# kevlar-dev/kevlar

Measured on AMD Instinct MI355X. Metric: reads/sec through count+novel (3 samples, k=31), higher is better.
Workload: dtype u64 hash / u8 counters

## Files before the change

### kevlar_amd/csrc/kv_skm.hip

```cpp
#include <algorithm>
#include <cmath>

#include "kv_binned.h"
#include "kv_novel_device.h"
#include "kv_skm_device.h"

struct SkmGeom {
    int k, m, w, wpow;
    int kw, nbw, recw, ncap;
    uint32_t C1, F2, fbits;
    uint32_t nwg1, nwg2, quota1;
    uint32_t cap1, cap2;
    uint32_t np_max;
    uint64_t stride;
    uint64_t *seg1; uint32_t *cnt1;
    uint64_t *seg2; uint32_t *cnt2;
    uint64_t *loose; uint64_t loose_cap;
    unsigned long long *ctr;
    uint32_t n_buckets, quota3;
    uint32_t sbw;
    uint64_t bucket_kmers;
    uint32_t force_loose;
    uint64_t *abl_keys; uint8_t *abl_cnts; uint32_t *abl_bstart, *abl_bcount; uint32_t abl_cap_wg;
    uint64_t *dl_keys, *dl_hash; uint32_t *dl_bstart, *dl_bcount; uint32_t dl_cap_wg;
// ... 636 lines not shown
        auto append = [&](unsigned long long bal, uint32_t v, uint32_t lane_start, uint32_t end) -> bool {
            const uint32_t slot = __builtin_amdgcn_mbcnt_hi((uint32_t)(bal >> 32), __builtin_amdgcn_mbcnt_lo((uint32_t)bal, n_ent));
            if (slot >= SKM_LANE_CAP) return false;
            ent[slot] = (unsigned long long)v | ((unsigned long long)(lane_start | (end << 18)) << 32);
            return true;
        };
        auto flush = [&]() {
            if (!pf_waited) {
#pragma unroll
                for (int i = 0; i < NW; ++i) asm volatile("" : "+v"(pf[i]));
                pf_waited = true;
            }
            __builtin_amdgcn_fence(__ATOMIC_ACQ_REL, "wavefront");
            __builtin_amdgcn_wave_barrier();
            const uint32_t n = min(n_ent, SKM_LANE_CAP);
            for (uint32_t e = lane; e < n; e += 64u) {
                const unsigned long long en = ent[e];
                const uint32_t hi = (uint32_t)(en >> 32), first = (hi >> 6) & 4095u;
                emit_run((uint32_t)en, hi & 63u, first, (hi >> 18) - first);
            }
            __builtin_amdgcn_fence(__ATOMIC_ACQ_REL, "wavefront");
            __builtin_amdgcn_wave_barrier();
            n_ent = 0;
        };
        uint32_t Sa[B], Sb[B];
#pragma unroll
        for (int j = 0; j < B; ++j) { Sa[j] = 0xffffffffu; Sb[j] = 0xffffffffu; }
        uint32_t prev_v = 0, start_prev = 0;
        const uint32_t rbase = lane * wpr;
        uint32_t since = 0;
        for (uint32_t b = 0; b < nblocks; b += (C == 2 ? 2u : 1u)) {
            skm_lane_block<C>(wl, rbase, lane, b, npos, nk, Sa, Sb, prev_v, start_prev, n_ent, append);
            if (C == 2 && b + 1u < nblocks) skm_lane_block<C>(wl, rbase, lane, b + 1u, npos, nk, Sb, Sa, prev_v, start_prev, n_ent, append);
            since += (C == 2 ? 2u : 1u);
            if ((since >= flush_blocks || n_ent + 192u > SKM_LANE_CAP) && n_ent && b + (C == 2 ? 2u : 1u) < nblocks) { flush(); since = 0; }
        }
        if (n_ent + 64u > SKM_LANE_CAP) flush();
        {
            const unsigned long long bal = __ballot(active);
            if (active) (void)append(bal, prev_v, start_prev, nk);
            n_ent += (uint32_t)__popcll(bal);
        }
        flush();
    }
    __syncthreads();
    for (uint32_t c = threadIdx.x; c < sg.C1; c += SKM_LANE_THREADS) sg.cnt1[skm_seg1_slot(sg, c, blockIdx.x)] = min(cur[c], sg.cap1);
    n_rec = wave_sum_u64(n_rec);
    if ((threadIdx.x & 63u) == 0 && n_rec) atomicAdd(&sg.ctr[SKM_CTR_RECORDS], (unsigned long long)n_rec);
}

#define SKM_THREADS2 512
#define SKM_MAX_F2 4096u
template <bool COMPACT>
__global__ __launch_bounds__(SKM_THREADS2) void k_skm_split(SkmGeom sg)
{
    __shared__ uint32_t cur[SKM_MAX_F2];
    __shared__ uint32_t spre[769];
    const uint32_t c = blockIdx.y;
    for (uint32_t f = threadIdx.x; f < sg.F2; f += SKM_THREADS2) cur[f] = 0;
    const uint32_t nmine = (skm_seg1_count(sg) - blockIdx.x + sg.nwg2 - 1) / sg.nwg2;
    for (uint32_t i = threadIdx.x; i < nmine; i += SKM_THREADS2) spre[i + 1] = sg.cnt1[skm_seg1_slot(sg, c, blockIdx.x + i * sg.nwg2)];
    __syncthreads();
    if (threadIdx.x == 0) {
        uint32_t acc = 0;
        for (uint32_t i = 0; i < nmine; ++i) { const uint32_t n = spre[i + 1]; spre[i] = acc; acc += n; }
        spre[nmine] = acc;
    }
    __syncthreads();
    const uint32_t total = spre[nmine];
    const int recw = COMPACT ? 2 : sg.recw;
    for (uint32_t i = threadIdx.x; i < total; i += SKM_THREADS2) {
        const uint32_t si = skm_search(spre, nmine, i);
        const uint32_t seg = blockIdx.x + si * sg.nwg2;
        const uint64_t *rec = sg.seg1 + (skm_seg1_first(sg, skm_seg1_slot(sg, c, seg)) + (i - spre[si])) * (uint64_t)recw;
        if (COMPACT) {
            typedef uint64_t u64x2a __attribute__((ext_vector_type(2), aligned(16)));
            const u64x2a both = *(const u64x2a *)rec;
            const uint32_t fine = skm_c_fine(both.y);
            const uint32_t p = atomicAdd(&cur[fine], 1u);
            if (p < sg.cap2) {
                *(u64x2a *)(sg.seg2 + ((((uint64_t)c * sg.F2 + fine) * sg.nwg2 + blockIdx.x) * sg.cap2 + p) * 2ull) = both;
            } else {
                uint64_t lw[3] = {both.x, skm_c_b1(both.y), 0ull};
                skm_loose_push(sg, skm_header(0ull, skm_c_n(both.y), fine, skm_c_rev(both.y)), lw);
            }
            continue;
        }
        const uint64_t hdr = rec[0];
        uint64_t bw[3];
#pragma unroll
        for (int t = 0; t < 3; ++t) bw[t] = t < sg.nbw ? rec[1 + t] : 0ull;
        const uint32_t fine = skm_hdr_fine(hdr);
        const uint32_t p = atomicAdd(&cur[fine], 1u);
        if (p < sg.cap2)
            skm_store_record(sg.seg2 + ((((uint64_t)c * sg.F2 + fine) * sg.nwg2 + blockIdx.x) * sg.cap2 + p) * (uint64_t)recw, hdr, bw, sg.nbw);
        else skm_loose_push(sg, hdr, bw);
    }
    __syncthreads();
    for (uint32_t f = threadIdx.x; f < sg.F2; f += SKM_THREADS2)
        sg.cnt2[((uint64_t)c * sg.F2 + f) * sg.nwg2 + blockIdx.x] = min(cur[f], sg.cap2);
}

#define SKM_S2_CHUNK 2048u
#define SKM_S2_MAXF 1024u
template <int RECW>
__global__ __launch_bounds__(SKM_THREADS2) void k_skm_split_sorted(SkmGeom sg)
{
    __shared__ uint32_t cur[SKM_S2_MAXF];
    __shared__ uint32_t hist[SKM_S2_MAXF];
    __shared__ uint32_t off[SKM_S2_MAXF];
    __shared__ uint32_t spre[769];
    __shared__ uint32_t wsum[SKM_THREADS2 / 64];
    extern __shared__ __attribute__((aligned(16))) uint64_t img[];
    const uint32_t c = blockIdx.y, F2 = sg.F2;
    const uint32_t lane = threadIdx.x & 63u, wave = threadIdx.x >> 6;
    for (uint32_t f = threadIdx.x; f < F2; f += SKM_THREADS2) { cur[f] = 0; hist[f] = 0; }
    const uint32_t nmine = (skm_seg1_count(sg) - blockIdx.x + sg.nwg2 - 1) / sg.nwg2;
    for (uint32_t i = threadIdx.x; i < nmine; i += SKM_THREADS2) spre[i + 1] = sg.cnt1[skm_seg1_slot(sg, c, blockIdx.x + i * sg.nwg2)];
    __syncthreads();
    if (threadIdx.x == 0) {
        uint32_t acc = 0;
        for (uint32_t i = 0; i < nmine; ++i) { const uint32_t n = spre[i + 1]; spre[i] = acc; acc += n; }
        spre[nmine] = acc;
    }
    __syncthreads();
    const uint32_t total = spre[nmine];
    constexpr uint32_t PER = SKM_S2_CHUNK / SKM_THREADS2;
    const uint32_t fper = (F2 + SKM_THREADS2 - 1) / SKM_THREADS2;
    uint64_t *const out = sg.seg2 + ((uint64_t)c * F2 * sg.nwg2 + blockIdx.x) * sg.cap2 * RECW;
    const uint64_t fstride = (uint64_t)sg.nwg2 * sg.cap2 * RECW;
    uint64_t nh[PER], n0[PER], n1[PER], n2[PER];
    auto request = [&](uint32_t c0) {
        const uint32_t n = c0 < total ? min(SKM_S2_CHUNK, total - c0) : 0u;
#pragma unroll
        for (uint32_t r = 0; r < PER; ++r) {
            const uint32_t i = r * SKM_THREADS2 + threadIdx.x;
            nh[r] = 0; n0[r] = 0; n1[r] = 0; n2[r] = 0;
            if (i < n) {
                const uint32_t gi = c0 + i, si = skm_search(spre, nmine, gi);
                const uint32_t seg = blockIdx.x + si * sg.nwg2;
                const uint64_t *rec = sg.seg1 + (skm_seg1_first(sg, skm_seg1_slot(sg, c, seg)) + (gi - spre[si])) * (uint64_t)RECW;
                if (RECW == 2) {
                    typedef uint64_t u64x2a __attribute__((ext_vector_type(2), aligned(16)));
                    const u64x2a both = *(const u64x2a *)rec;
                    n0[r] = both.x; nh[r] = both.y;
                } else {
                    nh[r] = rec[0]; n0[r] = rec[1]; n1[r] = rec[2];
                    if (RECW == 4) n2[r] = rec[3];
                }
            }
        }
    };
    request(0);
    for (uint32_t c0 = 0; c0 < total; c0 += SKM_S2_CHUNK) {
        const uint32_t n = min(SKM_S2_CHUNK, total - c0);
        uint64_t hdr[PER], w0[PER], w1[PER], w2[PER];
        uint32_t rank[PER];
#pragma unroll
        for (uint32_t r = 0; r < PER; ++r) { hdr[r] = nh[r]; w0[r] = n0[r]; w1[r] = n1[r]; w2[r] = n2[r]; rank[r] = 0; }
        request(c0 + SKM_S2_CHUNK);
#pragma unroll
        for (uint32_t r = 0; r < PER; ++r)
            if (r * SKM_THREADS2 + threadIdx.x < n) rank[r] = atomicAdd(&hist[RECW == 2 ? skm_c_fine(hdr[r]) : skm_hdr_fine(hdr[r])], 1u);
        __syncthreads();
        {
            uint32_t h[2] = {0, 0}, sum = 0;
            for (uint32_t j = 0; j < fper; ++j) {
                const uint32_t f = threadIdx.x * fper + j;
                h[j] = f < F2 ? hist[f] : 0u;
                sum += h[j];
            }
            uint32_t incl = sum;
#pragma unroll
            for (int d = 1; d < 64; d <<= 1) {
                const uint32_t up = __shfl_up(incl, d);
                if (lane >= (uint32_t)d) incl += up;
            }
            if (lane == 63) wsum[wave] = incl;
            __syncthreads();
            uint32_t before = incl - sum;
            for (uint32_t wv = 0; wv < wave; ++wv) before += wsum[wv];
            for (uint32_t j = 0; j < fper; ++j) {
                const uint32_t f = threadIdx.x * fper + j;
                if (f < F2) {
                    off[f] = before;
                    const uint32_t at = cur[f];
                    cur[f] = at + h[j];
                    hist[f] = at - before;
                    before += h[j];
                }
            }
        }
        __syncthreads();
#pragma unroll
        for (uint32_t r = 0; r < PER; ++r) {
            if (r * SKM_THREADS2 + threadIdx.x < n) {
                uint64_t *dst = img + (uint64_t)(off[RECW == 2 ? skm_c_fine(hdr[r]) : skm_hdr_fine(hdr[r])] + rank[r]) * RECW;
                if (RECW == 2) { dst[0] = w0[r]; dst[1] = hdr[r]; }
                else { dst[0] = hdr[r]; dst[1] = w0[r]; dst[2] = w1[r]; }
                if (RECW == 4) dst[3] = w2[r];
            }
        }
        __syncthreads();
        for (uint32_t wd = threadIdx.x; wd < n * RECW; wd += SKM_THREADS2) {
            const uint32_t q = wd / RECW, part = wd - q * RECW;
            const uint64_t h0 = img[(uint64_t)q * RECW + (RECW == 2 ? 1 : 0)];
            const uint32_t f = RECW == 2 ? skm_c_fine(h0) : skm_hdr_fine(h0);
            const uint32_t slot = q + hist[f];
            if (slot < sg.cap2) out[(uint64_t)f * fstride + (uint64_t)slot * RECW + part] = img[wd];
            else if (part == 0) {
                if (RECW == 2) {
                    uint64_t bw[3] = {img[(uint64_t)q * RECW], skm_c_b1(h0), 0ull};
                    skm_loose_push(sg, skm_header(0ull, skm_c_n(h0), f, skm_c_rev(h0)), bw);
                } else {
                    uint64_t bw[3] = {img[(uint64_t)q * RECW + 1], img[(uint64_t)q * RECW + 2], RECW == 4 ? img[(uint64_t)q * RECW + 3] : 0ull};
                    skm_loose_push(sg, h0, bw);
                }
            }
        }
        __syncthreads();
        for (uint32_t f = threadIdx.x; f < F2; f += SKM_THREADS2) hist[f] = 0;
        __syncthreads();
    }
    for (uint32_t f = threadIdx.x; f < F2; f += SKM_THREADS2)
        sg.cnt2[((uint64_t)c * F2 + f) * sg.nwg2 + blockIdx.x] = min(cur[f], sg.cap2);
}

#define SKM_STEP_MASK 62u
#define SKM_PROBE_STEP(h) ((((h) >> 20) & SKM_STEP_MASK) | 1u)
template <int TS>
__device__ __forceinline__ uint32_t skm_slot0(uint32_t sh) { return (TS & (TS - 1)) == 0 ? sh & (uint32_t)(TS - 1) : __umulhi(sh, (uint32_t)TS); }
template <int TS>
__device__ __forceinline__ uint32_t skm_step_of(uint32_t sh) { return (TS & (TS - 1)) == 0 ? SKM_PROBE_STEP(sh) : (((sh >> 2) & 62u) | 1u); }
template <int TS>
__device__ __forceinline__ uint32_t skm_slot_next(uint32_t slot, uint32_t step)
{
    if ((TS & (TS - 1)) == 0) return (slot + step) & (uint32_t)(TS - 1);
    slot += step;
    return slot >= (uint32_t)TS ? slot - (uint32_t)TS : slot;
}
template <int KW, int TS>
struct SkmTable {
    unsigned long long key[KW][TS];
};

template <int KW, int TS>
__device__ __forceinline__ void skm_table_clear(SkmTable<KW, TS> &tb)
{
    for (uint32_t i = threadIdx.x; i < TS; i += blockDim.x) {
        tb.key[0][i] = SKM_EMPTY;
        if (KW == 2) tb.key[KW - 1][i] = SKM_EMPTY;
    }
}

template <int KW, int TS>
__device__ __forceinline__ int skm_table_insert(SkmTable<KW, TS> &tb, const SkmKey<KW> &c)
{
    const uint32_t sh = skm_slot_hash<KW>(c);
    uint32_t slot = skm_slot0<TS>(sh);
    const uint32_t step = skm_step_of<TS>(sh);
    for (int probe = 0; probe < SKM_MAXPROBE; ++probe) {
        const unsigned long long old0 = atomicCAS(&tb.key[0][slot], SKM_EMPTY, (unsigned long long)c.w[0]);
        if (old0 == SKM_EMPTY || old0 == c.w[0]) {
            if (KW == 1) return (int)slot;
            const unsigned long long old1 = atomicCAS(&tb.key[KW - 1][slot], SKM_EMPTY, (unsigned long long)c.w[KW - 1]);
            if (old1 == SKM_EMPTY || old1 == c.w[KW - 1]) return (int)slot;
        }
        slot = skm_slot_next<TS>(slot, step);
    }
    return -1;
}

template <int KW, int TS>
__device__ __forceinline__ int skm_table_find(const SkmTable<KW, TS> &tb, const SkmKey<KW> &c)
{
    const uint32_t sh = skm_slot_hash<KW>(c);
    uint32_t slot = skm_slot0<TS>(sh);
    const uint32_t step = skm_step_of<TS>(sh);
    for (int probe = 0; probe < SKM_MAXPROBE; ++probe) {
        const unsigned long long k0 = tb.key[0][slot];
        if (k0 == SKM_EMPTY) return -1;
        if (k0 == c.w[0] && (KW == 1 || tb.key[KW - 1][slot] == c.w[KW - 1])) return (int)slot;
        slot = skm_slot_next<TS>(slot, step);
    }
    return -1;
}

template <typename Emit>
__device__ __forceinline__ uint32_t skm_count_kmer(uint64_t h, uint32_t count, const SketchDev *__restrict__ sk,
                                                   const SketchDev *__restrict__ mask, const ConsumeFilter &f, int T, Emit emit)
{
    if (!consume_filter_pass(f, mask, h)) return 0;
    uint32_t left = min(count, 255u);
    while (left) {
        const uint32_t wgt = min(left, BIN_W_MAX);
#pragma unroll
        for (int t = 0; t < BIN_MAX_T; ++t)
            if (t < T) emit(t, fastmod(h, sk->size[t], sk->magic[t]), wgt);
        left -= wgt;
    }
    return count;
}

template <int TS, typename Body>
__device__ __forceinline__ void skm_for_occupied(const unsigned long long *key0, uint16_t *queue_all, uint32_t queue_stride, Body body, const uint32_t *skip = nullptr)
{
    const uint32_t wave = threadIdx.x >> 6, lane = threadIdx.x & 63, nwaves = blockDim.x >> 6;
    uint16_t *queue = queue_all + wave * queue_stride;
    const uint32_t per_wave = TS / nwaves;
    const uint32_t s_end = (wave + 1) * per_wave;
    uint32_t qn = 0;
    for (uint32_t s0 = wave * per_wave;; s0 += 64) {
        const bool last = s0 >= s_end;
        if (!last) {
            const uint32_t slot = s0 + lane;
            const bool occ = key0[slot] != SKM_EMPTY && !(skip && ((skip[slot >> 5] >> (slot & 31u)) & 1u));
            const unsigned long long ballot = __ballot(occ);
            if (occ) __hip_atomic_store(&queue[qn + (uint32_t)__popcll(ballot & ((1ull << lane) - 1ull))], (uint16_t)slot, __ATOMIC_RELAXED, __HIP_MEMORY_SCOPE_WAVEFRONT);
            qn += (uint32_t)__popcll(ballot);
            __builtin_amdgcn_fence(__ATOMIC_ACQ_REL, "wavefront");
            __builtin_amdgcn_wave_barrier();
        }
        if (qn >= 64 || (last && qn > 0)) {
            const uint32_t take = min(qn, 64u);
            qn -= take;
            if (lane < take) body((uint32_t)__hip_atomic_load(&queue[qn + lane], __ATOMIC_RELAXED, __HIP_MEMORY_SCOPE_WAVEFRONT));
            __builtin_amdgcn_fence(__ATOMIC_ACQ_REL, "wavefront");
            __builtin_amdgcn_wave_barrier();
        }
        if (last) break;
    }
}

#define SKM_UNIT 4

__device__ __forceinline__ uint64_t skm_shfl64(uint64_t v, uint32_t src)
{
    const uint32_t lo = (uint32_t)__shfl((int)(uint32_t)v, (int)src), hi = (uint32_t)__shfl((int)(uint32_t)(v >> 32), (int)src);
    return (uint64_t)lo | ((uint64_t)hi << 32);
}

template <int KW>
__device__ __forceinline__ SkmKey<KW> skm_kmer_at(uint64_t b0, uint64_t b1, uint64_t b2, uint32_t j, int k)
{
    return skm_kmer_of<KW>(b0, b1, b2, j, k);
}

template <int KW, bool WANT_POS>
__device__ __forceinline__ void skm_walk_loose(const SkmGeom &sg, bool alone, const SkmKey<KW> &kmer, uint64_t hdr, uint32_t owner,
                                               uint64_t pos0, uint32_t j0, uint32_t u, uint32_t lane, int recw)
{
    const unsigned long long need = __ballot(alone);
    if (!need) return;
    const uint64_t posu = WANT_POS ? pos0 : skm_hdr_pos_of(skm_shfl64(hdr, owner), j0 + u);
    unsigned long long first = 0;
    if (lane == 0) first = atomicAdd(&sg.ctr[SKM_CTR_LOOSE], (unsigned long long)__popcll(need));
    first = skm_shfl64(first, 0);
    if (alone) {
        const unsigned long long idx = first + (unsigned long long)__popcll(need & ((1ull << lane) - 1ull));
        uint64_t one[3] = {kmer.w[0], KW == 2 ? kmer.w[KW - 1] : 0ull, 0ull};
        if (idx < sg.loose_cap) skm_store_record(sg.loose + idx * (uint64_t)recw, skm_header(posu, 1u, 0u), one, sg.nbw);
        else sg.ctr[SKM_CTR_FAIL] = 1;
    }
}

template <int KW, bool WANT_POS, int FK = 0, bool COMPACT = false, typename Body>
__device__ __forceinline__ void skm_walk_bucket(const SkmGeom &sg, uint32_t b, uint32_t *sbits_all, Body body)
{
    static_assert(!COMPACT || (KW == 1 && !WANT_POS), "compact records: one-word keys, no positions");
    constexpr uint32_t G = SKM_UNIT;
    const uint32_t lane = threadIdx.x & 63, wave = threadIdx.x >> 6, nwaves = blockDim.x >> 6;
    uint32_t *sbits = sbits_all + wave * sg.sbw;
    const int k = FK ? FK : sg.k, recw = COMPACT ? 2 : (FK ? 1 + KW + 1 : sg.recw);
    auto load = [&](const uint64_t *rec, uint64_t &hdr, uint64_t &b0, uint64_t &b1, uint64_t &b2) {
        if (COMPACT) {
            typedef uint64_t u64x2a __attribute__((ext_vector_type(2), aligned(16)));
            const u64x2a both = *(const u64x2a *)rec;
            b0 = both.x; b1 = skm_c_b1(both.y); hdr = skm_header(0ull, skm_c_n(both.y), 0u, skm_c_rev(both.y));
        } else {
            hdr = rec[0]; b0 = rec[1]; b1 = rec[2];
            if (KW == 2) b2 = rec[3];
        }
    };
    const uint32_t *cnt2 = sg.cnt2 + (uint64_t)b * sg.nwg2;
    uint32_t p = wave;
    uint32_t g = p / sg.nwg2, sgm = p - g * sg.nwg2;
    uint64_t hdr = 0, b0 = 0, b1 = 0, b2 = 0;
    {
        const uint32_t at = min(g * 64u + lane, sg.cap2 - 1u);
        const uint64_t *rec = sg.seg2 + (((uint64_t)b * sg.nwg2 + sgm) * sg.cap2 + at) * (uint64_t)recw;
        load(rec, hdr, b0, b1, b2);
    }
    uint32_t maxc = 0;
    for (uint32_t s2 = 0; s2 < sg.nwg2; ++s2) maxc = max(maxc, cnt2[s2]);
    for (;;) {
        if (g * 64u >= maxc) break;
        const uint32_t NR = cnt2[sgm], i = g * 64u + lane;
        const uint32_t nk = i < NR ? skm_hdr_n(hdr) : 0u;
        const uint32_t nu = (nk + G - 1u) / G;
        uint32_t incl = nu;
#pragma unroll
        for (int d = 1; d < 64; d <<= 1) {
            const uint32_t up = __shfl_up(incl, d);
            if (lane >= d) incl += up;
        }
        const uint32_t total = __shfl(incl, 63), excl = incl - nu;
        const uint32_t exnk = excl | (nk << 16);
        const uint32_t nwords = (total >> 5) + 2u;
        for (uint32_t wd = lane; wd < nwords; wd += 64) sbits[wd] = 0;
        __builtin_amdgcn_fence(__ATOMIC_RELEASE, "wavefront");
        __builtin_amdgcn_wave_barrier();
        if (nu) atomicOr(&sbits[excl >> 5], 1u << (excl & 31));
        __builtin_amdgcn_fence(__ATOMIC_ACQ_REL, "wavefront");
        __builtin_amdgcn_wave_barrier();
        uint32_t before = 0;
        for (uint32_t t0 = 0; t0 < total; t0 += 64) {
            const uint64_t starts = (uint64_t)__hip_atomic_load(&sbits[t0 >> 5], __ATOMIC_RELAXED, __HIP_MEMORY_SCOPE_WAVEFRONT) |
                                    ((uint64_t)__hip_atomic_load(&sbits[(t0 >> 5) + 1], __ATOMIC_RELAXED, __HIP_MEMORY_SCOPE_WAVEFRONT) << 32);
            const uint32_t t = t0 + lane;
            const uint32_t owner = (before + (uint32_t)__popcll(starts & ((2ull << lane) - 1ull)) - 1u) & 63u;
            before += (uint32_t)__popcll(starts);
            const uint32_t oe = (uint32_t)__shfl((int)exnk, (int)owner);
            const uint64_t o0 = skm_shfl64(b0, owner), o1 = skm_shfl64(b1, owner);
            const uint64_t o2 = KW == 2 ? skm_shfl64(b2, owner) : 0ull;
            const uint64_t oh = WANT_POS ? skm_shfl64(hdr, owner) : 0ull;
            const uint32_t j0 = t < total ? (t - (oe & 0xffffu)) * G : 0u;
            const uint32_t cnt = t < total ? min(G, (oe >> 16) - j0) : 0u;
            SkmKey<KW> fw = skm_kmer_of<KW>(o0, o1, o2, j0, k);
            const uint32_t tail = (uint32_t)skm_window64(o0, o1, o2, j0 + (uint32_t)k);
            uint64_t pos0 = 0;
            int step = 1;
            if (WANT_POS) {
                const bool rv = skm_hdr_rev(oh) != 0u;
                pos0 = skm_hdr_pos(oh) + (rv ? skm_hdr_n(oh) - 1u - j0 : j0);
                step = rv ? -1 : 1;
            }
#pragma unroll
            for (uint32_t u = 0; u < G; ++u) {
                if (u) { SkmKey<KW> other = fw; skm_roll<KW>(fw, other, (tail >> (2u * (u - 1u))) & 3u, k); }
                const uint64_t posu = pos0 + (uint64_t)(int64_t)(step * (int)u);
                bool alone = false;
                if (u < cnt) alone = body(fw, posu);
                skm_walk_loose<KW, WANT_POS>(sg, alone, fw, hdr, owner, posu, j0, u, lane, sg.lrecw);
            }
        }
        __builtin_amdgcn_wave_barrier();
        p += nwaves;
        g = p / sg.nwg2; sgm = p - g * sg.nwg2;
        if (g * 64u >= maxc) break;
        if (g * 64u + lane < cnt2[sgm]) {
            const uint64_t *rec = sg.seg2 + (((uint64_t)b * sg.nwg2 + sgm) * sg.cap2 + g * 64u + lane) * (uint64_t)recw;
            load(rec, hdr, b0, b1, b2);
        }
    }
}

__host__ __device__ inline uint32_t skm_wave_scratch_words(uint32_t sbw) { return sbw > 64u ? sbw : 64u; }

#define SKM_K2_WAVES 6
#define SKM_TS51 2560
#define SKM_TS31 4096
#define SKM_LIST_MAX 4096u
template <int KW, int TS, bool FORCE_LOOSE, int FK, bool COMPACT = false>
__global__ __launch_bounds__(SKM_THREADS3, KW == 2 ? SKM_K2_WAVES : 6) void k_skm_count(SkmGeom sg, const SketchDev *__restrict__ sk,
                                                           const SketchDev *__restrict__ mask, ConsumeFilter f, BinGeom g)
{
    static_assert((uint32_t)TS <= SKM_LIST_MAX, "a bucket's distinct list (one entry per occupied slot) must fit what k_skm_novel_list takes");
    constexpr bool PL = FK != 0;
    __shared__ SkmTable<KW, TS> tb;
    __shared__ uint32_t cnt[PL ? TS / 2 : TS];
    __shared__ uint32_t next_bucket;
    __shared__ uint32_t abl_cur, abl_b0, abl_prev;
    __shared__ uint32_t dl_cur, dl_b0;
    extern __shared__ __attribute__((aligned(16))) uint32_t dyn[];
    const uint32_t ns = (uint32_t)(g.T * g.C);
    uint32_t *lut = dyn, *cur = dyn + (PL ? 1024 : 256), *scratch = cur + ((ns + 3u) & ~3u);
    uint64_t *P1 = (uint64_t *)dyn, *P2 = P1 + 256;
    for (uint32_t s = threadIdx.x; s < ns; s += SKM_THREADS3) cur[s] = 0;
    if (threadIdx.x < 256) {
        if (PL) { P1[threadIdx.x] = skm_ascii4_times(threadIdx.x, MM_C1); P2[threadIdx.x] = skm_ascii4_times(threadIdx.x, MM_C2); }
        else lut[threadIdx.x] = skm_ascii4(threadIdx.x);
    }
    const HashParams hp = FK ? make_hash_params(FK, f.hp.hashfam) : f.hp;
    uint64_t n_added = 0, n_distinct = 0;
    const uint32_t cap1 = (uint32_t)g.cap1;
    uint32_t *my_seg = g.gbuf1 + (uint64_t)blockIdx.x * g.cap1;
    const uint64_t seg_stride = (uint64_t)g.nwgA * g.cap1;
    auto emit = [&](int t, uint64_t bin, uint32_t wgt) {
        const uint32_t slice = (uint32_t)(bin >> g.sbits);
        const uint32_t c = g.F == 1 ? slice : __umulhi(slice, g.recipF);
        const uint32_t sidx = (uint32_t)t * (uint32_t)g.C + c;
        const uint32_t item = ((slice - c * (uint32_t)g.F) << g.sbits) | ((uint32_t)bin & ((1u << g.sbits) - 1u)) | ((wgt - 1u) << BIN_W_SHIFT);
        const uint32_t pos = atomicAdd(&cur[sidx], 1u);
        if (pos < cap1) my_seg[sidx * seg_stride + pos] = item;
        else spill_item(g, t, bin, wgt);
    };
    skm_table_clear(tb);
    for (uint32_t i = threadIdx.x; i < (PL ? TS / 2 : TS); i += SKM_THREADS3) cnt[i] = 0;
    if (threadIdx.x == 0) { next_bucket = (uint32_t)atomicAdd(&sg.ctr[SKM_CTR_TICKET_COUNT], 1ull) * sg.bpt; abl_cur = 0; abl_b0 = 0; abl_prev = 0xffffffffu; dl_cur = 0; dl_b0 = 0; }
    auto abl_close = [&]() {
        if (sg.abl_keys && abl_prev != 0xffffffffu) {
            const bool fits = abl_cur <= sg.abl_cap_wg;
            sg.abl_bstart[abl_prev] = blockIdx.x * sg.abl_cap_wg + abl_b0;
            sg.abl_bcount[abl_prev] = fits ? abl_cur - abl_b0 : 0u;
        }
        if (sg.dl_keys && abl_prev != 0xffffffffu) {
            sg.dl_bstart[abl_prev] = blockIdx.x * sg.dl_cap_wg + dl_b0;
            sg.dl_bcount[abl_prev] = dl_cur - dl_b0;
        }
    };
    for (uint32_t taken = 0; taken < sg.quota3; ++taken) {
        __syncthreads();
        const uint32_t b = next_bucket;
        if (b >= sg.n_buckets) break;
        __syncthreads();
        if (threadIdx.x == 0) {
            abl_close();
            abl_prev = b; abl_b0 = abl_cur; dl_b0 = dl_cur;
            if ((b + 1u) & (sg.bpt - 1u)) next_bucket = b + 1u;
            else if (taken + 1 >= sg.quota3 || __hip_atomic_load(&sg.ctr[SKM_CTR_FAIL], __ATOMIC_RELAXED, __HIP_MEMORY_SCOPE_AGENT) != 0) next_bucket = 0xffffffffu;
            else {
                const unsigned long long ticket = atomicAdd(&sg.ctr[SKM_CTR_TICKET_COUNT], 1ull);
                next_bucket = (uint32_t)ticket * sg.bpt;
                const unsigned long long done = ticket * sg.bpt;
                if (done * 50ull >= sg.n_buckets) {
                    const unsigned long long now = __hip_atomic_load(&sg.ctr[SKM_CTR_LOOSE], __ATOMIC_RELAXED, __HIP_MEMORY_SCOPE_AGENT), start = sg.ctr[SKM_CTR_LOOSE_S12];
                    if (now > start && (now - start) * 25ull > done * sg.bucket_kmers) sg.ctr[SKM_CTR_FAIL] = 1;
                }
            }
        }
        skm_walk_bucket<KW, false, FK, COMPACT>(sg, b, scratch, [&](const SkmKey<KW> &c, uint64_t) {
            const bool forced = FORCE_LOOSE && sg.force_loose && ((c.w[0] * 0x9e3779b97f4a7c15ull) >> 58) == 0;
            const int slot = skm_cacheable<KW>(c) && !forced ? skm_table_insert(tb, c) : -1;
            if (slot >= 0) {
                if (PL) atomicAdd(&cnt[(uint32_t)slot >> 1], 1u << (((uint32_t)slot & 1u) * 16u));
                else atomicAdd(&cnt[slot], 1u);
            }
            return slot < 0;
        });
        __syncthreads();
        skm_for_occupied<TS>(tb.key[0], (uint16_t *)scratch, skm_wave_scratch_words(sg.sbw) * 2u, [&](uint32_t slot) {
            SkmKey<KW> c;
            c.w[0] = tb.key[0][slot];
            tb.key[0][slot] = SKM_EMPTY;
            if (KW == 2) { c.w[KW - 1] = tb.key[KW - 1][slot]; tb.key[KW - 1][slot] = SKM_EMPTY; }
            uint32_t seen;
            if (PL) {
                const uint32_t sh = (slot & 1u) * 16u;
                seen = (cnt[slot >> 1] >> sh) & 0xffffu;
                atomicSub(&cnt[slot >> 1], seen << sh);
            } else {
                seen = cnt[slot];
                cnt[slot] = 0;
            }
            n_distinct += 1;
            uint64_t h;
            if constexpr (PL) h = skm_key_hash_pl<KW, FK>(c, P1, P2);
            else h = skm_key_hash<KW>(c, lut, hp);
            if (sg.dl_keys) {
                const unsigned long long here = __ballot(true);
                const uint32_t lane = threadIdx.x & 63u, leader = (uint32_t)__ffsll((long long)here) - 1u;
                uint32_t base = 0;
                if (lane == leader) base = atomicAdd(&dl_cur, (uint32_t)__popcll(here));
                base = (uint32_t)__shfl((int)base, (int)leader);
                const uint32_t at = base + (uint32_t)__popcll(here & ((1ull << lane) - 1ull));
                if (at < sg.dl_cap_wg) {
                    const uint64_t e = (uint64_t)blockIdx.x * sg.dl_cap_wg + at;
                    sg.dl_keys[e * KW] = c.w[0];
                    if (KW == 2) sg.dl_keys[e * KW + (KW - 1)] = c.w[KW - 1];
                    sg.dl_hash[e] = h;
                }
            }
            uint32_t added;
            if (g.fast4 && !f.use_mask) {
                const bool pass = !f.use_band || (h >= f.band_lo && h < f.band_hi);
                added = pass ? seen : 0u;
                if (pass) {
                    const double hd = kv_fastmod_hd(h);
                    uint32_t bin[4];
#pragma unroll
                    for (int t = 0; t < 4; ++t) bin[t] = kv_fastmod32(h, hd, (uint32_t)g.tsize[t], g.tmagic[t]);
                    uint32_t left = min(seen, 255u);
                    const uint32_t omask = (1u << g.sbits) - 1u, stride32 = (uint32_t)seg_stride;
                    while (left) {
                        const uint32_t wgt = min(left, BIN_W_MAX), wbits = (wgt - 1u) << BIN_W_SHIFT;
#pragma unroll
                        for (int t = 0; t < 4; ++t) {
                            const uint32_t slice = bin[t] >> g.sbits;
                            const uint32_t c = g.F == 1 ? slice : __umulhi(slice, g.recipF);
                            const uint32_t sidx = (uint32_t)t * (uint32_t)g.C + c;
                            const uint32_t item = ((slice - c * (uint32_t)g.F) << g.sbits) | (bin[t] & omask) | wbits;
                            const uint32_t pos = atomicAdd(&cur[sidx], 1u);
                            if (pos < cap1) my_seg[sidx * stride32 + pos] = item;
                            else spill_item(g, t, (uint64_t)bin[t], wgt);
                        }
                        left -= wgt;
                    }
                }
            } else {
                added = skm_count_kmer(h, seen, sk, mask, f, g.T, emit);
            }
            n_added += added;
            if (sg.abl_keys) {
                const bool want = added >= 2u;
                const unsigned long long here = __ballot(true), vote = __ballot(want);
                if (vote) {
                    const uint32_t lane = threadIdx.x & 63u, leader = (uint32_t)__ffsll((long long)here) - 1u;
                    uint32_t base = 0;
                    if (lane == leader) base = atomicAdd(&abl_cur, (uint32_t)__popcll(vote));
                    base = (uint32_t)__shfl((int)base, (int)leader);
                    const uint32_t at = base + (uint32_t)__popcll(vote & ((1ull << lane) - 1ull));
                    if (want && at < sg.abl_cap_wg) {
                        const uint64_t e = (uint64_t)blockIdx.x * sg.abl_cap_wg + at;
                        sg.abl_keys[e * KW] = c.w[0];
                        if (KW == 2) sg.abl_keys[e * KW + (KW - 1)] = c.w[KW - 1];
                        sg.abl_cnts[e] = (uint8_t)min(added, 255u);
                    }
                }
            }
        });
    }
    __syncthreads();
    if (threadIdx.x == 0) {
        abl_close();
        if (sg.dl_keys && dl_cur > sg.dl_cap_wg) atomicAdd(&sg.ctr[SKM_CTR_DL_RAN_OUT], 1ull);
    }
    for (uint32_t s = threadIdx.x; s < ns; s += SKM_THREADS3)
        g.gcnt1[(uint64_t)s * g.nwgA + blockIdx.x] = (uint32_t)min((uint64_t)cur[s], g.cap1);
    n_added = wave_sum_u64(n_added);
    n_distinct = wave_sum_u64(n_distinct);
    if ((threadIdx.x & 63) == 0 && n_added) atomicAdd(&g.ctr[BIN_CTR_ADDED], (unsigned long long)n_added);
    if ((threadIdx.x & 63) == 0 && n_distinct) atomicAdd(&sg.ctr[SKM_CTR_DISTINCT], (unsigned long long)n_distinct);
}

template <int KW>
__global__ __launch_bounds__(256) void k_skm_loose_count(SkmGeom sg, const SketchDev *__restrict__ sk,
                                                         const SketchDev *__restrict__ mask, ConsumeFilter f, BinGeom g)
{
    __shared__ uint32_t lut[256];
    if (sg.ctr[SKM_CTR_FAIL] != 0) return;
    lut[threadIdx.x] = skm_ascii4(threadIdx.x);
    __syncthreads();
    unsigned long long n = sg.ctr[SKM_CTR_LOOSE];
    if (n > sg.loose_cap) n = sg.loose_cap;
    const int k = sg.k, recw = sg.lrecw;
    uint64_t n_added = 0;
    const uint64_t stride = (uint64_t)gridDim.x * blockDim.x;
    const uint32_t lane = threadIdx.x & 63u;
    auto count_one = [&](const SkmKey<KW> &fw, bool live) {
        uint64_t h = 0;
        bool pass = false;
        if (live) {
            h = skm_key_hash<KW>(skm_canonical<KW>(fw, skm_revcomp<KW>(fw, k)), lut, f.hp);
            pass = consume_filter_pass(f, mask, h);
        }
        n_added += pass ? 1 : 0;
        uint64_t bins[BIN_MAX_T];
#pragma unroll
        for (int t = 0; t < BIN_MAX_T; ++t) bins[t] = (pass && t < g.T) ? fastmod(h, sk->size[t], sk->magic[t]) : 0ull;
        spill_items_wave(g, bins, 1u, pass);
    };
    const uint64_t total_waves = (uint64_t)gridDim.x * (blockDim.x >> 6), wave_id = (uint64_t)blockIdx.x * (blockDim.x >> 6) + (threadIdx.x >> 6);
    const uint32_t per = (uint32_t)min((unsigned long long)64, max((unsigned long long)1, (n + total_waves - 1) / total_waves));
    (void)stride;
    for (uint64_t i0 = wave_id * per; i0 < n; i0 += total_waves * per) {
        const uint64_t i = i0 + lane;
        const bool have = lane < per && i < n;
        const uint64_t *rec = sg.loose + (have ? i : 0) * (uint64_t)recw;
        uint64_t bw[3];
#pragma unroll
        for (int t = 0; t < 3; ++t) bw[t] = (have && t < sg.nbw) ? rec[1 + t] : 0ull;
        const uint32_t nk = have ? skm_hdr_n(rec[0]) : 0u;
        count_one(skm_first_kmer<KW>(bw, k), nk == 1);
        unsigned long long longer = __ballot(nk > 1);
        while (longer) {
            const uint32_t src = (uint32_t)__ffsll((long long)longer) - 1u;
            longer &= longer - 1ull;
            const uint64_t b0 = skm_shfl64(bw[0], src), b1 = skm_shfl64(bw[1], src), b2 = skm_shfl64(bw[2], src);
            const uint32_t nk_src = (uint32_t)__shfl((int)nk, (int)src);
            for (uint32_t j0 = 0; j0 < nk_src; j0 += 64) {
                const uint32_t j = j0 + lane;
                const bool live = j < nk_src;
                count_one(skm_kmer_at<KW>(b0, b1, b2, live ? j : 0u, k), live);
            }
        }
    }
    n_added = wave_sum_u64(n_added);
    if ((threadIdx.x & 63) == 0 && n_added) atomicAdd(&g.ctr[BIN_CTR_ADDED], (unsigned long long)n_added);
}

#define SKM_ROUTE_MAX_DEST 16
struct SkmOverflowSink { unsigned long long *ctr; uint64_t *ovf; uint8_t *ovf_dest; uint64_t ovf_cap; int ndest; };
__device__ __attribute__((noinline)) void skm_route_overflow(SkmOverflowSink rs, uint32_t d, uint64_t h, uint64_t count)
{
    {
        const unsigned long long here = __ballot(true);
        const uint32_t lane = threadIdx.x & 63u, leader = (uint32_t)__ffsll((long long)here) - 1u;
        unsigned long long o = 0;
        if (lane == leader) o = atomicAdd(&rs.ctr[ROUTE_CTR_OVERFLOW], (unsigned long long)__popcll(here));
        o = skm_shfl64(o, leader) + (unsigned long long)__popcll(here & ((1ull << lane) - 1ull));
        const bool fits = o < rs.ovf_cap;
        for (int dd = 0; dd < rs.ndest; ++dd) {
            const unsigned long long same = __ballot(fits && d == (uint32_t)dd);
            if (same && lane == (uint32_t)__ffsll((long long)same) - 1u) atomicAdd(&rs.ctr[ROUTE_CTR_DEST0 + dd], (unsigned long long)__popcll(same));
        }
        if (fits) {
            *(ulonglong2 *)(rs.ovf + 2 * o) = make_ulonglong2(h, count);
            rs.ovf_dest[o] = (uint8_t)d;
        }
    }
}

__device__ __forceinline__ void skm_route_item(const KvRouteSink &rs, const uint64_t *lo, uint32_t *cur, uint64_t h, uint64_t count)
{
    if (h == UINT64_MAX) return;
    uint32_t d = 0;
    for (int b = 1; b < rs.ndest; ++b) d += h >= lo[b] ? 1u : 0u;
    const uint32_t pos = cur ? atomicAdd(&cur[d], 1u) : 0xffffffffu;
    if (pos < rs.seg_cap) *(ulonglong2 *)(rs.seg + (((uint64_t)d * rs.nwg + blockIdx.x) * rs.seg_cap + pos) * 2) = make_ulonglong2(h, count);
    else skm_route_overflow(SkmOverflowSink{rs.ctr, rs.ovf, rs.ovf_dest, rs.ovf_cap, rs.ndest}, d, h, count);
}

template <int KW, int TS, bool COMPACT = false>
__global__ __launch_bounds__(SKM_THREADS3, 6) void k_skm_route(SkmGeom sg, HashParams hp, KvRouteSink rs)
{
    __shared__ SkmTable<KW, TS> tb;
    __shared__ uint32_t cnt[TS];
    __shared__ uint32_t next_bucket;
    __shared__ uint32_t cur[SKM_ROUTE_MAX_DEST];
    __shared__ uint64_t lo[SKM_ROUTE_MAX_DEST];
    __shared__ uint32_t dl_cur, dl_b0, dl_prev;
    __shared__ uint32_t dl_org, dl_lim;
    extern __shared__ __attribute__((aligned(16))) uint32_t dyn[];
    uint32_t *lut = dyn, *scratch = dyn + 256;
    if (threadIdx.x < 256) lut[threadIdx.x] = skm_ascii4(threadIdx.x);
    if (threadIdx.x < (uint32_t)rs.ndest) { cur[threadIdx.x] = 0; lo[threadIdx.x] = rs.bs * (uint64_t)threadIdx.x; }
    const int k = sg.k;
    uint64_t n_distinct = 0;
    skm_table_clear(tb);
    for (uint32_t i = threadIdx.x; i < TS; i += SKM_THREADS3) cnt[i] = 0;
    if (threadIdx.x == 0) {
        next_bucket = (uint32_t)atomicAdd(&sg.ctr[SKM_CTR_TICKET_COUNT], 1ull) * sg.bpt; dl_cur = 0; dl_b0 = 0; dl_prev = 0xffffffffu;
        dl_org = sg.dl_chunk ? 0u : blockIdx.x * sg.dl_cap_wg; dl_lim = sg.dl_chunk ? 0u : sg.dl_cap_wg;
    }
    auto dl_close = [&]() {
        if (sg.dl_keys && dl_prev != 0xffffffffu) {
            sg.dl_bstart[dl_prev] = dl_org + dl_b0;
            sg.dl_bcount[dl_prev] = dl_cur - dl_b0;
            if (sg.dl_chunk && dl_cur > dl_lim) atomicAdd(&sg.ctr[SKM_CTR_DL_RAN_OUT], 1ull);
        }
    };
    auto passes_of = [&](uint32_t b) {
        const uint32_t least = sg.passes > 1u ? sg.passes : 1u;
        const uint32_t *cnt2 = sg.cnt2 + (uint64_t)b * sg.nwg2;
        uint32_t nrec = 0;
        for (uint32_t s2 = 0; s2 < sg.nwg2; ++s2) nrec += cnt2[s2];
        const uint32_t per_pass = (uint32_t)TS * 13u / 20u;
        const uint32_t want = (19u * nrec / 10u + per_pass - 1u) / per_pass;
        return min(64u, max(least, want));
    };
    for (uint32_t taken = 0; taken < sg.quota3; ++taken) {
        __syncthreads();
        const uint32_t b = next_bucket;
        if (b >= sg.n_buckets) break;
        __syncthreads();
        if (threadIdx.x == 0) {
            dl_close();
            if (sg.dl_keys && sg.dl_chunk) {
                const uint32_t need = passes_of(b) * (uint32_t)TS;
                if (dl_cur + need > dl_lim) {
                    const unsigned long long c = atomicAdd(&sg.ctr[SKM_CTR_POOL_CHUNKS], 1ull);
                    if (c < sg.dl_nchunks && need <= sg.dl_chunk) { dl_org = (uint32_t)c * sg.dl_chunk; dl_lim = sg.dl_chunk; }
                    else { dl_org = 0; dl_lim = 0; atomicAdd(&sg.ctr[SKM_CTR_DL_RAN_OUT], 1ull); }
                    dl_cur = 0;
                }
            }
            dl_prev = b; dl_b0 = dl_cur;
            if ((b + 1u) & (sg.bpt - 1u)) next_bucket = b + 1u;
            else if (taken + 1 >= sg.quota3 || __hip_atomic_load(&sg.ctr[SKM_CTR_FAIL], __ATOMIC_RELAXED, __HIP_MEMORY_SCOPE_AGENT) != 0) next_bucket = 0xffffffffu;
            else next_bucket = (uint32_t)atomicAdd(&sg.ctr[SKM_CTR_TICKET_COUNT], 1ull) * sg.bpt;
        }
        const uint32_t passes = passes_of(b);
        for (uint32_t pass = 0; pass < passes; ++pass) {
        if (pass) __syncthreads();
        skm_walk_bucket<KW, false, 0, COMPACT>(sg, b, scratch, [&](const SkmKey<KW> &c, uint64_t) {
            if (!skm_cacheable<KW>(c)) return pass == 0u;
            if (passes > 1u && __umulhi(skm_slot_hash<KW>(c) * 0x9E3779B1u, passes) != pass) return false;
            const int slot = skm_table_insert(tb, c);
            if (slot >= 0) atomicAdd(&cnt[slot], 1u);
            return slot < 0;
        });
        __syncthreads();
        skm_for_occupied<TS>(tb.key[0], (uint16_t *)scratch, skm_wave_scratch_words(sg.sbw) * 2u, [&](uint32_t slot) {
            SkmKey<KW> c;
            c.w[0] = tb.key[0][slot];
            tb.key[0][slot] = SKM_EMPTY;
            if (KW == 2) { c.w[KW - 1] = tb.key[KW - 1][slot]; tb.key[KW - 1][slot] = SKM_EMPTY; }
            const uint32_t seen = cnt[slot];
            cnt[slot] = 0;
            n_distinct += 1;
            const uint64_t h = skm_key_hash<KW>(c, lut, hp);
            if (sg.dl_keys) {
                const unsigned long long here = __ballot(true);
                const uint32_t lane = threadIdx.x & 63u, leader = (uint32_t)__ffsll((long long)here) - 1u;
                uint32_t base = 0;
                if (lane == leader) base = atomicAdd(&dl_cur, (uint32_t)__popcll(here));
                base = (uint32_t)__shfl((int)base, (int)leader);
                const uint32_t at = base + (uint32_t)__popcll(here & ((1ull << lane) - 1ull));
                if (at < dl_lim) {
                    const uint64_t e = (uint64_t)dl_org + at;
                    sg.dl_keys[e * KW] = c.w[0];
                    if (KW == 2) sg.dl_keys[e * KW + (KW - 1)] = c.w[KW - 1];
                    sg.dl_hash[e] = h;
                }
            }
            skm_route_item(rs, lo, cur, h, seen);
        });
        }
    }
    __syncthreads();
    if (threadIdx.x == 0) {
        dl_close();
        if (sg.dl_keys && !sg.dl_chunk && dl_cur > sg.dl_cap_wg) atomicAdd(&sg.ctr[SKM_CTR_DL_RAN_OUT], 1ull);
    }
    if (threadIdx.x < (uint32_t)rs.ndest)
        rs.seg_count[(uint64_t)threadIdx.x * rs.nwg + blockIdx.x] = (uint32_t)min((uint64_t)cur[threadIdx.x], rs.seg_cap);
    n_distinct = wave_sum_u64(n_distinct);
    if ((threadIdx.x & 63) == 0 && n_distinct) atomicAdd(&sg.ctr[SKM_CTR_DISTINCT], (unsigned long long)n_distinct);
}

template <int KW>
__global__ __launch_bounds__(256) void k_skm_loose_route(SkmGeom sg, HashParams hp, KvRouteSink rs)
{
    __shared__ uint32_t lut[256];
    __shared__ uint64_t lo[SKM_ROUTE_MAX_DEST];
    __shared__ uint32_t dcount[SKM_ROUTE_MAX_DEST];
    __shared__ uint32_t wg_items, wg_cur;
    __shared__ unsigned long long wg_base;
    if (sg.ctr[SKM_CTR_FAIL] != 0) return;
    lut[threadIdx.x] = skm_ascii4(threadIdx.x);
    if (threadIdx.x < SKM_ROUTE_MAX_DEST) { lo[threadIdx.x] = rs.bs * (uint64_t)threadIdx.x; dcount[threadIdx.x] = 0; }
    if (threadIdx.x == 0) { wg_items = 0; wg_cur = 0; }
    __syncthreads();
    unsigned long long n = sg.ctr[SKM_CTR_LOOSE];
// ... 1430 lines not shown
```

Measured before the change: 992.7 million.

## Pool leftover occupied slots across waves for load-balanced drain in skm_for_occupied

The occupied-slot iteration is restructured so each wave processes a full batch as soon as its queue reaches 64 entries, rather than using a separate drain step. With POOL enabled (single-word keys), leftover partial queues from all waves are published to shared memory and redistributed in 64-wide batches across waves, so several waves no longer each run a partially filled final body call. This is meant to cut divergent, underfilled tail work in the per-bucket emit phase. It adds a block-wide __syncthreads and a small per-lane owner search over waves, and it depends on every wave reaching the barrier.

Result: no change. 1.000 billion (median of 2 runs) (+0.8%).

```diff
diff --git a/kevlar_amd/csrc/kv_skm.hip b/kevlar_amd/csrc/kv_skm.hip
--- a/kevlar_amd/csrc/kv_skm.hip
+++ b/kevlar_amd/csrc/kv_skm.hip
@@ -962,33 +962,60 @@
     return count;
 }
 
-template <int TS, typename Body>
+template <int TS, bool POOL = false, typename Body>
 __device__ __forceinline__ void skm_for_occupied(const unsigned long long *key0, uint16_t *queue_all, uint32_t queue_stride, Body body, const uint32_t *skip = nullptr)
 {
-    const uint32_t wave = threadIdx.x >> 6, lane = threadIdx.x & 63, nwaves = blockDim.x >> 6;
+    __shared__ uint32_t left_n[SKM_THREADS3 / 64];
+    const uint32_t wave = (uint32_t)__builtin_amdgcn_readfirstlane((int)(threadIdx.x >> 6)), lane = threadIdx.x & 63, nwaves = blockDim.x >> 6;
     uint16_t *queue = queue_all + wave * queue_stride;
     const uint32_t per_wave = TS / nwaves;
     const uint32_t s_end = (wave + 1) * per_wave;
     uint32_t qn = 0;
-    for (uint32_t s0 = wave * per_wave;; s0 += 64) {
-        const bool last = s0 >= s_end;
-        if (!last) {
-            const uint32_t slot = s0 + lane;
-            const bool occ = key0[slot] != SKM_EMPTY && !(skip && ((skip[slot >> 5] >> (slot & 31u)) & 1u));
+    uint32_t s0 = wave * per_wave, batch = wave;
+    bool pooled = false;
+    for (;;) {
+        uint32_t slot = 0;
+        bool have = false;
+        if (s0 < s_end) {
+            const uint32_t at = s0 + lane;
+            const bool occ = key0[at] != SKM_EMPTY && !(skip && ((skip[at >> 5] >> (at & 31u)) & 1u));
             const unsigned long long ballot = __ballot(occ);
-            if (occ) __hip_atomic_store(&queue[qn + (uint32_t)__popcll(ballot & ((1ull << lane) - 1ull))], (uint16_t)slot, __ATOMIC_RELAXED, __HIP_MEMORY_SCOPE_WAVEFRONT);
+            if (occ) __hip_atomic_store(&queue[qn + (uint32_t)__popcll(ballot & ((1ull << lane) - 1ull))], (uint16_t)at, __ATOMIC_RELAXED, __HIP_MEMORY_SCOPE_WAVEFRONT);
             qn += (uint32_t)__popcll(ballot);
+            s0 += 64;
             __builtin_amdgcn_fence(__ATOMIC_ACQ_REL, "wavefront");
             __builtin_amdgcn_wave_barrier();
-        }
-        if (qn >= 64 || (last && qn > 0)) {
-            const uint32_t take = min(qn, 64u);
-            qn -= take;
-            if (lane < take) body((uint32_t)__hip_atomic_load(&queue[qn + lane], __ATOMIC_RELAXED, __HIP_MEMORY_SCOPE_WAVEFRONT));
-            __builtin_amdgcn_fence(__ATOMIC_ACQ_REL, "wavefront");
-            __builtin_amdgcn_wave_barrier();
-        }
-        if (last) break;
+            if (qn >= 64) {
+                qn -= 64;
+                slot = (uint32_t)__hip_atomic_load(&queue[qn + lane], __ATOMIC_RELAXED, __HIP_MEMORY_SCOPE_WAVEFRONT);
+                have = true;
+            }
+        } else if (!POOL) {
+            if (pooled || qn == 0) break;
+            pooled = true;
+            have = lane < qn;
+            if (have) slot = (uint32_t)__hip_atomic_load(&queue[lane], __ATOMIC_RELAXED, __HIP_MEMORY_SCOPE_WAVEFRONT);
+        } else {
+            if (!pooled) {
+                if (lane == 0) left_n[wave] = qn;
+                __syncthreads();
+                pooled = true;
+            }
+            const uint32_t idx = batch * 64u + lane;
+            uint32_t total = 0, owner = 0, off = 0;
+            for (uint32_t w = 0; w < nwaves; ++w) {
+                const uint32_t c = left_n[w];
+                if (idx >= total && idx - total < c) { owner = w; off = idx - total; }
+                total += c;
+            }
+            if (batch * 64u >= total) break;
+            have = idx < total;
+            if (have) slot = (uint32_t)queue_all[owner * queue_stride + off];
+            batch += nwaves;
+        }
+        if (have) body(slot);
+        __builtin_amdgcn_fence(__ATOMIC_ACQ_REL, "wavefront");
+        __builtin_amdgcn_wave_barrier();
     }
 }
 
@@ -1199,7 +1226,7 @@
             return slot < 0;
         });
         __syncthreads();
-        skm_for_occupied<TS>(tb.key[0], (uint16_t *)scratch, skm_wave_scratch_words(sg.sbw) * 2u, [&](uint32_t slot) {
+        skm_for_occupied<TS, KW == 1>(tb.key[0], (uint16_t *)scratch, skm_wave_scratch_words(sg.sbw) * 2u, [&](uint32_t slot) {
             SkmKey<KW> c;
             c.w[0] = tb.key[0][slot];
             tb.key[0][slot] = SKM_EMPTY;
```
